# facebookresearch/multimodal

Hardware: NVIDIA H100
Metric: image-text pairs/sec (CLIP ViT-B/16 contrastive pretrain step, bs=512/GPU) (higher is better)
Workload: dtype bf16

## Files before the change

multimodal_b200/csrc/attention.cu:

```cuda
#include "common.cuh"
#include "mmb200_internal.h"
#include <stdlib.h>

namespace mmb {

constexpr int HD = 64;
constexpr int SMAX = 384;

__device__ __forceinline__ uint32_t toff(int r, int c) { return (uint32_t)(r * 128 + ((((c >> 3) ^ (r & 7))) << 4)); }

__device__ __forceinline__ void load_a(uint32_t (&a)[4], uint32_t base, int r0, int c0, int lane) {
  ldsm_x4(a, base + toff(r0 + (lane & 7) + ((lane >> 3) & 1) * 8, c0 + (lane >> 4) * 8));
}
__device__ __forceinline__ void load_b_nk(uint32_t (&b)[4], uint32_t base, int n0, int k0, int lane) {
  ldsm_x4(b, base + toff(n0 + (lane & 7), k0 + (lane >> 3) * 8));
}
__device__ __forceinline__ void load_b_kn(uint32_t (&b)[4], uint32_t base, int k0, int n0, int lane) {
  ldsm_x4_t(b, base + toff(k0 + (lane & 7) + ((lane >> 3) & 1) * 8, n0 + (lane >> 4) * 8));
}

__device__ __forceinline__ void load_tile(uint8_t* dst, const __nv_bfloat16* src, long long ld, int S, int S_pad) {
  for (int i = threadIdx.x; i < S_pad * 8; i += blockDim.x) {
    const int r = i >> 3, ch = i & 7;
    uint4 v = make_uint4(0, 0, 0, 0);
    if (r < S) v = __ldg(reinterpret_cast<const uint4*>(src + (long long)r * ld + ch * 8));
    *reinterpret_cast<uint4*>(dst + toff(r, ch * 8)) = v;
  }
}
__device__ __forceinline__ void load_keymask(uint8_t* dst, const uint8_t* kmask, int S, int S_pad) {
  for (int i = threadIdx.x; i < S_pad; i += blockDim.x) dst[i] = (i < S && (!kmask || kmask[i])) ? 1 : 0;
}

__device__ __forceinline__ float quad_max(float v) {
  v = fmaxf(v, __shfl_xor_sync(0xffffffffu, v, 1));
  return fmaxf(v, __shfl_xor_sync(0xffffffffu, v, 2));
}
__device__ __forceinline__ float quad_sum(float v) {
  v += __shfl_xor_sync(0xffffffffu, v, 1);
  return v + __shfl_xor_sync(0xffffffffu, v, 2);
}

template <bool CAUSAL>
__global__ void __launch_bounds__(256) attn_fwd_kernel(const __nv_bfloat16* __restrict__ qkv,
                                                       __nv_bfloat16* __restrict__ out, float* __restrict__ lse,
                                                       const uint8_t* __restrict__ kmask, int S, int H,
                                                       float scale_log2) {
  extern __shared__ __align__(128) uint8_t asmem[];
  const int S_pad = (S + 15) & ~15;
  const int d = H * HD;
  const long long ld = 3LL * d;
  const int b = blockIdx.x / H, h = blockIdx.x - b * H;
  uint8_t* sQ = asmem;
  uint8_t* sK = sQ + S_pad * 128;
  uint8_t* sV = sK + S_pad * 128;
  uint8_t* sM = sV + S_pad * 128;
  const __nv_bfloat16* base = qkv + (long long)b * S * ld + h * HD;
  load_tile(sQ, base, ld, S, S_pad);
  load_tile(sK, base + d, ld, S, S_pad);
  load_tile(sV, base + 2 * d, ld, S, S_pad);
  load_keymask(sM, kmask ? kmask + (long long)b * S : nullptr, S, S_pad);
  __syncthreads();
  const uint32_t uQ = smem_u32(sQ), uK = smem_u32(sK), uV = smem_u32(sV);
  const int warp = threadIdx.x >> 5, lane = threadIdx.x & 31, nwarps = blockDim.x >> 5;
  const int g = lane >> 2, t = lane & 3;
  const int n_qt = S_pad >> 4;

  for (int qt = warp; qt < n_qt; qt += nwarps) {
    const int q0 = qt * 16;
    uint32_t qa[4][4];
#pragma unroll
    for (int ks = 0; ks < 4; ++ks) load_a(qa[ks], uQ, q0, ks * 16, lane);
    float o[8][4];
#pragma unroll
    for (int i = 0; i < 8; ++i) o[i][0] = o[i][1] = o[i][2] = o[i][3] = 0.f;
    float m0 = -INFINITY, m1 = -INFINITY, l0 = 0.f, l1 = 0.f;
    const int r0 = q0 + g, r1 = r0 + 8;
    const int kv_end = CAUSAL ? min(S, q0 + 16) : S;

    for (int kvb = 0; kvb < kv_end; kvb += 64) {
      const int nt_valid = min(8, (kv_end - kvb + 7) >> 3);
      float s[8][4];
#pragma unroll
      for (int nt = 0; nt < 8; ++nt) {
        s[nt][0] = s[nt][1] = s[nt][2] = s[nt][3] = 0.f;
        if (nt < nt_valid) {
#pragma unroll
          for (int kp = 0; kp < 2; ++kp) {
            uint32_t kb[4];
            load_b_nk(kb, uK, kvb + nt * 8, kp * 32, lane);
            mma16816(s[nt], qa[2 * kp], kb[0], kb[1]);
            mma16816(s[nt], qa[2 * kp + 1], kb[2], kb[3]);
          }
        }
      }
      float mx0 = -INFINITY, mx1 = -INFINITY;
#pragma unroll
      for (int nt = 0; nt < 8; ++nt) {
#pragma unroll
        for (int e = 0; e < 4; ++e) {
          const int col = kvb + nt * 8 + 2 * t + (e & 1);
          const int row = (e < 2) ? r0 : r1;
          float v = s[nt][e] * scale_log2;
          if (col >= kv_end || !sM[col] || (CAUSAL && col > row)) v = -INFINITY;
          s[nt][e] = v;
        }
        mx0 = fmaxf(mx0, fmaxf(s[nt][0], s[nt][1]));
        mx1 = fmaxf(mx1, fmaxf(s[nt][2], s[nt][3]));
      }
      mx0 = quad_max(mx0);
      mx1 = quad_max(mx1);
      const float mn0 = fmaxf(m0, mx0), mn1 = fmaxf(m1, mx1);
      const float b0 = (mn0 == -INFINITY) ? 0.f : mn0, b1 = (mn1 == -INFINITY) ? 0.f : mn1;
      const float c0 = exp2f(m0 - b0), c1 = exp2f(m1 - b1);
      float rs0 = 0.f, rs1 = 0.f;
#pragma unroll
      for (int nt = 0; nt < 8; ++nt) {
        s[nt][0] = exp2f(s[nt][0] - b0);
        s[nt][1] = exp2f(s[nt][1] - b0);
        s[nt][2] = exp2f(s[nt][2] - b1);
        s[nt][3] = exp2f(s[nt][3] - b1);
        rs0 += s[nt][0] + s[nt][1];
        rs1 += s[nt][2] + s[nt][3];
      }
      l0 = l0 * c0 + rs0;
      l1 = l1 * c1 + rs1;
      m0 = mn0;
      m1 = mn1;
#pragma unroll
      for (int i = 0; i < 8; ++i) {
        o[i][0] *= c0; o[i][1] *= c0; o[i][2] *= c1; o[i][3] *= c1;
      }
#pragma unroll
      for (int ks = 0; ks < 4; ++ks) {
        if (2 * ks < nt_valid) {
          uint32_t pa[4];
          pa[0] = pack_bf16x2(s[2 * ks][0], s[2 * ks][1]);
          pa[1] = pack_bf16x2(s[2 * ks][2], s[2 * ks][3]);
          pa[2] = pack_bf16x2(s[2 * ks + 1][0], s[2 * ks + 1][1]);
          pa[3] = pack_bf16x2(s[2 * ks + 1][2], s[2 * ks + 1][3]);
#pragma unroll
          for (int np = 0; np < 4; ++np) {
            uint32_t vb[4];
            load_b_kn(vb, uV, kvb + ks * 16, np * 16, lane);
            mma16816(o[2 * np], pa, vb[0], vb[1]);
            mma16816(o[2 * np + 1], pa, vb[2], vb[3]);
          }
        }
      }
    }
    l0 = quad_sum(l0);
    l1 = quad_sum(l1);
    const float i0 = l0 > 0.f ? 1.f / l0 : 0.f, i1 = l1 > 0.f ? 1.f / l1 : 0.f;
    __nv_bfloat16* orow0 = out + ((long long)b * S + r0) * d + h * HD;
    __nv_bfloat16* orow1 = out + ((long long)b * S + r1) * d + h * HD;
#pragma unroll
    for (int nt = 0; nt < 8; ++nt) {
      if (r0 < S) *reinterpret_cast<uint32_t*>(orow0 + nt * 8 + 2 * t) = pack_bf16x2(o[nt][0] * i0, o[nt][1] * i0);
      if (r1 < S) *reinterpret_cast<uint32_t*>(orow1 + nt * 8 + 2 * t) = pack_bf16x2(o[nt][2] * i1, o[nt][3] * i1);
    }
    if (lse && t == 0) {
      float* lrow = lse + ((long long)b * H + h) * S;
      if (r0 < S) lrow[r0] = (m0 + log2f(l0)) * 0.6931471805599453f;
      if (r1 < S) lrow[r1] = (m1 + log2f(l1)) * 0.6931471805599453f;
    }
  }
}

template <bool CAUSAL>
__global__ void __launch_bounds__(256) attn_bwd_kernel(const __nv_bfloat16* __restrict__ qkv,
                                                       const __nv_bfloat16* __restrict__ out,
                                                       const __nv_bfloat16* __restrict__ dout,
                                                       const float* __restrict__ lse,
                                                       const uint8_t* __restrict__ kmask,
                                                       __nv_bfloat16* __restrict__ dqkv, int S, int H, float scale) {
  extern __shared__ __align__(128) uint8_t asmem[];
  const int S_pad = (S + 15) & ~15;
  const int d = H * HD;
  const long long ld = 3LL * d;
  const int b = blockIdx.x / H, h = blockIdx.x - b * H;
  uint8_t* sQ = asmem;
  uint8_t* sK = sQ + S_pad * 128;
  uint8_t* sV = sK + S_pad * 128;
  uint8_t* sdO = sV + S_pad * 128;
  float* sL = reinterpret_cast<float*>(sdO + S_pad * 128);
  float* sD = sL + S_pad;
  uint8_t* sM = reinterpret_cast<uint8_t*>(sD + S_pad);
  const __nv_bfloat16* base = qkv + (long long)b * S * ld + h * HD;
  const __nv_bfloat16* obase = out + (long long)b * S * d + h * HD;
  const __nv_bfloat16* dobase = dout + (long long)b * S * d + h * HD;
  load_tile(sQ, base, ld, S, S_pad);
  load_tile(sK, base + d, ld, S, S_pad);
  load_tile(sV, base + 2 * d, ld, S, S_pad);
  load_tile(sdO, dobase, d, S, S_pad);
  load_keymask(sM, kmask ? kmask + (long long)b * S : nullptr, S, S_pad);
  const int warp = threadIdx.x >> 5, lane = threadIdx.x & 31, nwarps = blockDim.x >> 5;
  for (int r = warp; r < S_pad; r += nwarps) {
    float acc = 0.f;
    if (r < S) {
      const uint32_t a = *reinterpret_cast<const uint32_t*>(obase + (long long)r * d + lane * 2);
      const uint32_t c = *reinterpret_cast<const uint32_t*>(dobase + (long long)r * d + lane * 2);
      acc = bf16_lo(a) * bf16_lo(c) + bf16_hi(a) * bf16_hi(c);
    }
#pragma unroll
    for (int o = 16; o > 0; o >>= 1) acc += __shfl_xor_sync(0xffffffffu, acc, o);
    if (lane == 0) {
      sD[r] = acc;
      sL[r] = (r < S) ? lse[((long long)b * H + h) * S + r] * 1.4426950408889634f : 0.f;
    }
  }
  __syncthreads();
  const uint32_t uQ = smem_u32(sQ), uK = smem_u32(sK), uV = smem_u32(sV), uO = smem_u32(sdO);
  const int g = lane >> 2, t = lane & 3;
  const int n_t = S_pad >> 4;
  const float scale_log2 = scale * 1.4426950408889634f;
  __nv_bfloat16* dbase = dqkv + (long long)b * S * ld + h * HD;

  for (int j = warp; j < n_t; j += nwarps) {
    const int kv0 = j * 16;
    uint32_t ka[4][4], va[4][4];
#pragma unroll
    for (int ks = 0; ks < 4; ++ks) {
      load_a(ka[ks], uK, kv0, ks * 16, lane);
      load_a(va[ks], uV, kv0, ks * 16, lane);
    }
    float dk[8][4], dv[8][4];
#pragma unroll
    for (int i = 0; i < 8; ++i) {
      dk[i][0] = dk[i][1] = dk[i][2] = dk[i][3] = 0.f;
      dv[i][0] = dv[i][1] = dv[i][2] = dv[i][3] = 0.f;
    }
    const bool kv_ok0 = sM[kv0 + g] != 0, kv_ok1 = sM[kv0 + g + 8] != 0;
    for (int i = CAUSAL ? j : 0; i < n_t; ++i) {
      const int q0 = i * 16;
      float st[2][4], dpt[2][4];
#pragma unroll
      for (int nt = 0; nt < 2; ++nt) {
        st[nt][0] = st[nt][1] = st[nt][2] = st[nt][3] = 0.f;
        dpt[nt][0] = dpt[nt][1] = dpt[nt][2] = dpt[nt][3] = 0.f;
#pragma unroll
        for (int kp = 0; kp < 2; ++kp) {
          uint32_t qb[4], ob[4];
          load_b_nk(qb, uQ, q0 + nt * 8, kp * 32, lane);
          mma16816(st[nt], ka[2 * kp], qb[0], qb[1]);
          mma16816(st[nt], ka[2 * kp + 1], qb[2], qb[3]);
          load_b_nk(ob, uO, q0 + nt * 8, kp * 32, lane);
          mma16816(dpt[nt], va[2 * kp], ob[0], ob[1]);
          mma16816(dpt[nt], va[2 * kp + 1], ob[2], ob[3]);
        }
      }
      float pT[2][4], dsT[2][4];
#pragma unroll
      for (int nt = 0; nt < 2; ++nt)
#pragma unroll
        for (int e = 0; e < 4; ++e) {
          const int kv = kv0 + g + (e >> 1) * 8;
          const int q = q0 + nt * 8 + 2 * t + (e & 1);
          const bool valid = ((e >> 1) ? kv_ok1 : kv_ok0) && (q < S) && (!CAUSAL || kv <= q);
          const float p = valid ? exp2f(st[nt][e] * scale_log2 - sL[q]) : 0.f;
          pT[nt][e] = p;
          dsT[nt][e] = p * (dpt[nt][e] - sD[q]) * scale;
        }
      uint32_t pa[4], dsa[4];
      pa[0] = pack_bf16x2(pT[0][0], pT[0][1]); pa[1] = pack_bf16x2(pT[0][2], pT[0][3]);
      pa[2] = pack_bf16x2(pT[1][0], pT[1][1]); pa[3] = pack_bf16x2(pT[1][2], pT[1][3]);
      dsa[0] = pack_bf16x2(dsT[0][0], dsT[0][1]); dsa[1] = pack_bf16x2(dsT[0][2], dsT[0][3]);
      dsa[2] = pack_bf16x2(dsT[1][0], dsT[1][1]); dsa[3] = pack_bf16x2(dsT[1][2], dsT[1][3]);
#pragma unroll
      for (int np = 0; np < 4; ++np) {
        uint32_t bb[4];
        load_b_kn(bb, uO, q0, np * 16, lane);
        mma16816(dv[2 * np], pa, bb[0], bb[1]);
        mma16816(dv[2 * np + 1], pa, bb[2], bb[3]);
        load_b_kn(bb, uQ, q0, np * 16, lane);
        mma16816(dk[2 * np], dsa, bb[0], bb[1]);
        mma16816(dk[2 * np + 1], dsa, bb[2], bb[3]);
      }
    }
    const int r0 = kv0 + g, r1 = r0 + 8;
#pragma unroll
    for (int nt = 0; nt < 8; ++nt) {
      if (r0 < S) {
        *reinterpret_cast<uint32_t*>(dbase + (long long)r0 * ld + d + nt * 8 + 2 * t) = pack_bf16x2(dk[nt][0], dk[nt][1]);
        *reinterpret_cast<uint32_t*>(dbase + (long long)r0 * ld + 2 * d + nt * 8 + 2 * t) = pack_bf16x2(dv[nt][0], dv[nt][1]);
      }
      if (r1 < S) {
        *reinterpret_cast<uint32_t*>(dbase + (long long)r1 * ld + d + nt * 8 + 2 * t) = pack_bf16x2(dk[nt][2], dk[nt][3]);
        *reinterpret_cast<uint32_t*>(dbase + (long long)r1 * ld + 2 * d + nt * 8 + 2 * t) = pack_bf16x2(dv[nt][2], dv[nt][3]);
      }
    }
  }

  for (int i = warp; i < n_t; i += nwarps) {
    const int q0 = i * 16;
    uint32_t qa[4][4], oa[4][4];
#pragma unroll
    for (int ks = 0; ks < 4; ++ks) {
      load_a(qa[ks], uQ, q0, ks * 16, lane);
      load_a(oa[ks], uO, q0, ks * 16, lane);
    }
    float dq[8][4];
#pragma unroll
    for (int n = 0; n < 8; ++n) dq[n][0] = dq[n][1] = dq[n][2] = dq[n][3] = 0.f;
    const int r0 = q0 + g, r1 = r0 + 8;
    const float L0 = sL[r0], L1 = sL[r1], D0 = sD[r0], D1 = sD[r1];
    const int j_end = CAUSAL ? i + 1 : n_t;
    for (int j = 0; j < j_end; ++j) {
      const int kv0 = j * 16;
      float s[2][4], dp[2][4];
#pragma unroll
      for (int nt = 0; nt < 2; ++nt) {
        s[nt][0] = s[nt][1] = s[nt][2] = s[nt][3] = 0.f;
        dp[nt][0] = dp[nt][1] = dp[nt][2] = dp[nt][3] = 0.f;
#pragma unroll
        for (int kp = 0; kp < 2; ++kp) {
          uint32_t kb[4], vb[4];
          load_b_nk(kb, uK, kv0 + nt * 8, kp * 32, lane);
          mma16816(s[nt], qa[2 * kp], kb[0], kb[1]);
          mma16816(s[nt], qa[2 * kp + 1], kb[2], kb[3]);
          load_b_nk(vb, uV, kv0 + nt * 8, kp * 32, lane);
          mma16816(dp[nt], oa[2 * kp], vb[0], vb[1]);
          mma16816(dp[nt], oa[2 * kp + 1], vb[2], vb[3]);
        }
      }
      float ds[2][4];
#pragma unroll
      for (int nt = 0; nt < 2; ++nt)
#pragma unroll
        for (int e = 0; e < 4; ++e) {
          const int row = (e < 2) ? r0 : r1;
          const int col = kv0 + nt * 8 + 2 * t + (e & 1);
          const bool valid = (row < S) && sM[col] && (!CAUSAL || col <= row);
          const float p = valid ? exp2f(s[nt][e] * scale_log2 - ((e < 2) ? L0 : L1)) : 0.f;
          ds[nt][e] = p * (dp[nt][e] - ((e < 2) ? D0 : D1)) * scale;
        }
      uint32_t dsa[4];
      dsa[0] = pack_bf16x2(ds[0][0], ds[0][1]); dsa[1] = pack_bf16x2(ds[0][2], ds[0][3]);
      dsa[2] = pack_bf16x2(ds[1][0], ds[1][1]); dsa[3] = pack_bf16x2(ds[1][2], ds[1][3]);
#pragma unroll
      for (int np = 0; np < 4; ++np) {
        uint32_t bb[4];
        load_b_kn(bb, uK, kv0, np * 16, lane);
        mma16816(dq[2 * np], dsa, bb[0], bb[1]);
        mma16816(dq[2 * np + 1], dsa, bb[2], bb[3]);
      }
    }
#pragma unroll
    for (int nt = 0; nt < 8; ++nt) {
      if (r0 < S) *reinterpret_cast<uint32_t*>(dbase + (long long)r0 * ld + nt * 8 + 2 * t) = pack_bf16x2(dq[nt][0], dq[nt][1]);
      if (r1 < S) *reinterpret_cast<uint32_t*>(dbase + (long long)r1 * ld + nt * 8 + 2 * t) = pack_bf16x2(dq[nt][2], dq[nt][3]);
    }
  }
}

static int pick_threads(int S) {
  const int n_t = (S + 15) / 16;
  const int per = (n_t + 7) / 8;
  return ((n_t + per - 1) / per) * 32;
}

static int attention_fwd_impl(const void* qkv, void* out, float* lse, const uint8_t* kmask, int B, int S, int H,
                              int causal, float scale, void* stream) {
  if (B <= 0 || S <= 0 || H <= 0 || S > SMAX) return MMB_ERR_UNSUPPORTED;
  const int S_pad = (S + 15) & ~15;
  const int smem = 3 * S_pad * 128 + S_pad;
  const float scale_log2 = scale * 1.4426950408889634f;
  cudaStream_t st = reinterpret_cast<cudaStream_t>(stream);
  auto kfn = causal ? attn_fwd_kernel<true> : attn_fwd_kernel<false>;
  cudaError_t e = cudaFuncSetAttribute(kfn, cudaFuncAttributeMaxDynamicSharedMemorySize, smem);
  if (e != cudaSuccess) return (int)e;
  kfn<<<B * H, pick_threads(S), smem, st>>>((const __nv_bfloat16*)qkv, (__nv_bfloat16*)out, lse, kmask, S, H, scale_log2);
  return (int)cudaGetLastError();
}

static int attention_bwd_impl(const void* qkv, const void* out, const void* dout, const float* lse, void* dqkv,
                              const uint8_t* kmask, int B, int S, int H, int causal, float scale, void* stream) {
  if (B <= 0 || S <= 0 || H <= 0 || S > SMAX) return MMB_ERR_UNSUPPORTED;
  const int S_pad = (S + 15) & ~15;
  const int smem = 4 * S_pad * 128 + 2 * S_pad * 4 + S_pad;
  cudaStream_t st = reinterpret_cast<cudaStream_t>(stream);
  auto kfn = causal ? attn_bwd_kernel<true> : attn_bwd_kernel<false>;
  cudaError_t e = cudaFuncSetAttribute(kfn, cudaFuncAttributeMaxDynamicSharedMemorySize, smem);
  if (e != cudaSuccess) return (int)e;
  kfn<<<B * H, pick_threads(S), smem, st>>>((const __nv_bfloat16*)qkv, (const __nv_bfloat16*)out,
                                            (const __nv_bfloat16*)dout, lse, kmask, (__nv_bfloat16*)dqkv, S, H, scale);
  return (int)cudaGetLastError();
}

}

using namespace mmb;

extern "C" int mmb_attention_bwd_launches(int) { return 1; }

extern "C" int mmb_attention_fwd(const void* qkv, void* out, float* lse, int B, int S, int H, int head_dim, int causal,
                                 float scale, void* stream) {
  if (head_dim != HD) return MMB_ERR_UNSUPPORTED;
  return attention_fwd_impl(qkv, out, lse, nullptr, B, S, H, causal, scale, stream);
}
extern "C" int mmb_attention_fwd_kmask(const void* qkv, void* out, float* lse, const unsigned char* kmask, int B, int S,
// ... 16 lines not shown
```

multimodal_b200/csrc/common.cuh:

```cuda
#pragma once
#include <cuda.h>
#include <cuda_bf16.h>
#include <cuda_runtime.h>
#include <stdint.h>
#include <stdio.h>

namespace mmb {

__device__ __forceinline__ uint32_t smem_u32(const void* p) {
  return static_cast<uint32_t>(__cvta_generic_to_shared(p));
}

__device__ __forceinline__ uint64_t global_timer_ns() {
  uint64_t t;
  asm volatile("mov.u64 %0, %%globaltimer;" : "=l"(t));
  return t;
}

#ifndef MMB_WATCHDOG_NS
#define MMB_WATCHDOG_NS 4000000000ull
#endif

__device__ __forceinline__ void mbar_init(uint64_t* bar, uint32_t count) {
  asm volatile("mbarrier.init.shared::cta.b64 [%0], %1;" ::"r"(smem_u32(bar)), "r"(count) : "memory");
// ... 163 lines not shown
        "+f"(d[32]), "+f"(d[33]), "+f"(d[34]), "+f"(d[35]), "+f"(d[36]), "+f"(d[37]), "+f"(d[38]), "+f"(d[39]),
        "+f"(d[40]), "+f"(d[41]), "+f"(d[42]), "+f"(d[43]), "+f"(d[44]), "+f"(d[45]), "+f"(d[46]), "+f"(d[47]),
        "+f"(d[48]), "+f"(d[49]), "+f"(d[50]), "+f"(d[51]), "+f"(d[52]), "+f"(d[53]), "+f"(d[54]), "+f"(d[55]),
        "+f"(d[56]), "+f"(d[57]), "+f"(d[58]), "+f"(d[59]), "+f"(d[60]), "+f"(d[61]), "+f"(d[62]), "+f"(d[63]),
        "+f"(d[64]), "+f"(d[65]), "+f"(d[66]), "+f"(d[67]), "+f"(d[68]), "+f"(d[69]), "+f"(d[70]), "+f"(d[71]),
        "+f"(d[72]), "+f"(d[73]), "+f"(d[74]), "+f"(d[75]), "+f"(d[76]), "+f"(d[77]), "+f"(d[78]), "+f"(d[79]),
        "+f"(d[80]), "+f"(d[81]), "+f"(d[82]), "+f"(d[83]), "+f"(d[84]), "+f"(d[85]), "+f"(d[86]), "+f"(d[87]),
        "+f"(d[88]), "+f"(d[89]), "+f"(d[90]), "+f"(d[91]), "+f"(d[92]), "+f"(d[93]), "+f"(d[94]), "+f"(d[95]),
        "+f"(d[96]), "+f"(d[97]), "+f"(d[98]), "+f"(d[99]), "+f"(d[100]), "+f"(d[101]), "+f"(d[102]), "+f"(d[103]),
        "+f"(d[104]), "+f"(d[105]), "+f"(d[106]), "+f"(d[107]), "+f"(d[108]), "+f"(d[109]), "+f"(d[110]), "+f"(d[111]),
        "+f"(d[112]), "+f"(d[113]), "+f"(d[114]), "+f"(d[115]), "+f"(d[116]), "+f"(d[117]), "+f"(d[118]), "+f"(d[119]),
        "+f"(d[120]), "+f"(d[121]), "+f"(d[122]), "+f"(d[123]), "+f"(d[124]), "+f"(d[125]), "+f"(d[126]), "+f"(d[127])
      : "l"(adesc), "l"(bdesc), "r"(accumulate), "n"(TA), "n"(TB));
}

template <int N>
__device__ __forceinline__ void setmaxnreg_dec() { asm volatile("setmaxnreg.dec.sync.aligned.u32 %0;" ::"n"(N)); }
template <int N>
__device__ __forceinline__ void setmaxnreg_inc() { asm volatile("setmaxnreg.inc.sync.aligned.u32 %0;" ::"n"(N)); }

__device__ __forceinline__ void ldsm_x4(uint32_t (&r)[4], uint32_t addr) {
  asm volatile("ldmatrix.sync.aligned.m8n8.x4.shared.b16 {%0,%1,%2,%3}, [%4];"
               : "=r"(r[0]), "=r"(r[1]), "=r"(r[2]), "=r"(r[3])
               : "r"(addr));
}
__device__ __forceinline__ void ldsm_x4_t(uint32_t (&r)[4], uint32_t addr) {
  asm volatile("ldmatrix.sync.aligned.m8n8.x4.trans.shared.b16 {%0,%1,%2,%3}, [%4];"
               : "=r"(r[0]), "=r"(r[1]), "=r"(r[2]), "=r"(r[3])
               : "r"(addr));
}
// ... 52 lines not shown
```

Before: 2546.

## Rewrite attention fwd/bwd with TMA loads and wgmma over 64-row query blocks

Replaces the mma.sync/ldmatrix attention kernels with Hopper wgmma (m64n64k16) kernels fed by TMA tile loads into 128B-swizzled shared memory, with per-chunk mbarriers. The grid is split across 64-row query blocks, and in backward across separate key-role and query-role CTAs, instead of one CTA per (batch, head). This gives more parallelism and lets tensor-core work start while later K/V chunks are still arriving. In exchange it adds more redundant K/V loads per CTA, serialised wgmma waits with no overlap between steps, and host-side tensor-map creation on every call.

```diff
diff --git a/multimodal_b200/csrc/attention.cu b/multimodal_b200/csrc/attention.cu
--- a/multimodal_b200/csrc/attention.cu
+++ b/multimodal_b200/csrc/attention.cu
@@ -6,29 +6,18 @@
 
 constexpr int HD = 64;
 constexpr int SMAX = 384;
-
-__device__ __forceinline__ uint32_t toff(int r, int c) { return (uint32_t)(r * 128 + ((((c >> 3) ^ (r & 7))) << 4)); }
-
-__device__ __forceinline__ void load_a(uint32_t (&a)[4], uint32_t base, int r0, int c0, int lane) {
-  ldsm_x4(a, base + toff(r0 + (lane & 7) + ((lane >> 3) & 1) * 8, c0 + (lane >> 4) * 8));
-}
-__device__ __forceinline__ void load_b_nk(uint32_t (&b)[4], uint32_t base, int n0, int k0, int lane) {
-  ldsm_x4(b, base + toff(n0 + (lane & 7), k0 + (lane >> 3) * 8));
-}
-__device__ __forceinline__ void load_b_kn(uint32_t (&b)[4], uint32_t base, int k0, int n0, int lane) {
-  ldsm_x4_t(b, base + toff(k0 + (lane & 7) + ((lane >> 3) & 1) * 8, n0 + (lane >> 4) * 8));
-}
-
-__device__ __forceinline__ void load_tile(uint8_t* dst, const __nv_bfloat16* src, long long ld, int S, int S_pad) {
-  for (int i = threadIdx.x; i < S_pad * 8; i += blockDim.x) {
-    const int r = i >> 3, ch = i & 7;
-    uint4 v = make_uint4(0, 0, 0, 0);
-    if (r < S) v = __ldg(reinterpret_cast<const uint4*>(src + (long long)r * ld + ch * 8));
-    *reinterpret_cast<uint4*>(dst + toff(r, ch * 8)) = v;
-  }
-}
-__device__ __forceinline__ void load_keymask(uint8_t* dst, const uint8_t* kmask, int S, int S_pad) {
-  for (int i = threadIdx.x; i < S_pad; i += blockDim.x) dst[i] = (i < S && (!kmask || kmask[i])) ? 1 : 0;
+constexpr int TROWS = 64;
+constexpr int TILE_BYTES = TROWS * HD * 2;
+constexpr int MAX_CHUNKS = SMAX / TROWS;
+constexpr float LOG2E = 1.4426950408889634f;
+
+__device__ __forceinline__ uint64_t desc_kmajor(const uint8_t* tile) { return make_smem_desc_sw128(smem_u32(tile), 16, 1024); }
+__device__ __forceinline__ uint64_t desc_mnmajor(const uint8_t* tile) { return make_smem_desc_sw128(smem_u32(tile), TILE_BYTES, 1024); }
+constexpr uint64_t KSTEP_K = 32 >> 4;
+constexpr uint64_t KSTEP_MN = 2048 >> 4;
+
+__device__ __forceinline__ uint8_t* align1024(uint8_t* p) {
+  return p + ((1024u - (smem_u32(p) & 1023u)) & 1023u);
 }
 
 __device__ __forceinline__ float quad_max(float v) {
@@ -40,349 +29,342 @@
   return v + __shfl_xor_sync(0xffffffffu, v, 2);
 }
 
+__device__ __forceinline__ void mma_abt(float (&acc)[32], const uint8_t* a, const uint8_t* b) {
+  const uint64_t ad = desc_kmajor(a), bd = desc_kmajor(b);
+#pragma unroll
+  for (int k = 0; k < 4; ++k) wgmma_m64n64k16_ss<0, 0>(acc, ad + k * KSTEP_K, bd + k * KSTEP_K, k > 0 ? 1u : 0u);
+}
+__device__ __forceinline__ void mma_pb(float (&acc)[32], const uint32_t (&p)[4][4], const uint8_t* b) {
+  const uint64_t bd = desc_mnmajor(b);
+#pragma unroll
+  for (int k = 0; k < 4; ++k) wgmma_m64n64k16_rs<1>(acc, p[k], bd + k * KSTEP_MN, 1u);
+}
+__device__ __forceinline__ void pack_a(uint32_t (&p)[4][4], const float (&x)[32]) {
+#pragma unroll
+  for (int k = 0; k < 4; ++k)
+#pragma unroll
+    for (int i = 0; i < 4; ++i) p[k][i] = pack_bf16x2(x[8 * k + 2 * i], x[8 * k + 2 * i + 1]);
+}
+
+__device__ __forceinline__ void load_keymask(uint8_t* dst, const uint8_t* kmask, int S, int n) {
+  for (int i = threadIdx.x; i < n; i += blockDim.x) dst[i] = (i < S && (!kmask || kmask[i])) ? 1 : 0;
+}
+
 template <bool CAUSAL>
-__global__ void __launch_bounds__(256) attn_fwd_kernel(const __nv_bfloat16* __restrict__ qkv,
+__global__ void __launch_bounds__(128) attn_fwd_kernel(const __grid_constant__ CUtensorMap tmQKV,
                                                        __nv_bfloat16* __restrict__ out, float* __restrict__ lse,
                                                        const uint8_t* __restrict__ kmask, int S, int H,
                                                        float scale_log2) {
-  extern __shared__ __align__(128) uint8_t asmem[];
-  const int S_pad = (S + 15) & ~15;
+  extern __shared__ uint8_t smem_raw[];
+  uint8_t* smem = align1024(smem_raw);
+  const int nblk = (S + TROWS - 1) / TROWS;
+  const int bh = blockIdx.x / nblk, qb = blockIdx.x - bh * nblk;
+  const int b = bh / H, h = bh - b * H;
   const int d = H * HD;
-  const long long ld = 3LL * d;
-  const int b = blockIdx.x / H, h = blockIdx.x - b * H;
-  uint8_t* sQ = asmem;
-  uint8_t* sK = sQ + S_pad * 128;
-  uint8_t* sV = sK + S_pad * 128;
-  uint8_t* sM = sV + S_pad * 128;
-  const __nv_bfloat16* base = qkv + (long long)b * S * ld + h * HD;
-  load_tile(sQ, base, ld, S, S_pad);
-  load_tile(sK, base + d, ld, S, S_pad);
-  load_tile(sV, base + 2 * d, ld, S, S_pad);
-  load_keymask(sM, kmask ? kmask + (long long)b * S : nullptr, S, S_pad);
+  const int q0 = qb * TROWS;
+  const int kv_end = CAUSAL ? min(S, q0 + TROWS) : S;
+  const int nkc = (kv_end + TROWS - 1) / TROWS;
+  uint8_t* sQ = smem;
+  uint8_t* sK = sQ + TILE_BYTES;
+  uint8_t* sV = sK + nblk * TILE_BYTES;
+  uint64_t* bar = reinterpret_cast<uint64_t*>(sV + nblk * TILE_BYTES);
+  uint8_t* sM = reinterpret_cast<uint8_t*>(bar + MAX_CHUNKS);
+
+  if (threadIdx.x == 0) {
+    tma_prefetch_desc(&tmQKV);
+    for (int c = 0; c < nkc; ++c) mbar_init(&bar[c], 1);
+    fence_mbar_init();
+    for (int c = 0; c < nkc; ++c) {
+      mbar_arrive_expect_tx(&bar[c], (c == 0 ? 3 : 2) * TILE_BYTES);
+      if (c == 0) tma_load_3d(&tmQKV, &bar[0], sQ, h * HD, q0, b);
+      tma_load_3d(&tmQKV, &bar[c], sK + c * TILE_BYTES, d + h * HD, c * TROWS, b);
+      tma_load_3d(&tmQKV, &bar[c], sV + c * TILE_BYTES, 2 * d + h * HD, c * TROWS, b);
+    }
+  }
+  load_keymask(sM, kmask ? kmask + (long long)b * S : nullptr, S, nkc * TROWS);
   __syncthreads();
-  const uint32_t uQ = smem_u32(sQ), uK = smem_u32(sK), uV = smem_u32(sV);
-  const int warp = threadIdx.x >> 5, lane = threadIdx.x & 31, nwarps = blockDim.x >> 5;
-  const int g = lane >> 2, t = lane & 3;
-  const int n_qt = S_pad >> 4;
-
-  for (int qt = warp; qt < n_qt; qt += nwarps) {
-    const int q0 = qt * 16;
-    uint32_t qa[4][4];
-#pragma unroll
-    for (int ks = 0; ks < 4; ++ks) load_a(qa[ks], uQ, q0, ks * 16, lane);
-    float o[8][4];
-#pragma unroll
-    for (int i = 0; i < 8; ++i) o[i][0] = o[i][1] = o[i][2] = o[i][3] = 0.f;
-    float m0 = -INFINITY, m1 = -INFINITY, l0 = 0.f, l1 = 0.f;
-    const int r0 = q0 + g, r1 = r0 + 8;
-    const int kv_end = CAUSAL ? min(S, q0 + 16) : S;
-
-    for (int kvb = 0; kvb < kv_end; kvb += 64) {
-      const int nt_valid = min(8, (kv_end - kvb + 7) >> 3);
-      float s[8][4];
-#pragma unroll
-      for (int nt = 0; nt < 8; ++nt) {
-        s[nt][0] = s[nt][1] = s[nt][2] = s[nt][3] = 0.f;
-        if (nt < nt_valid) {
-#pragma unroll
-          for (int kp = 0; kp < 2; ++kp) {
-            uint32_t kb[4];
-            load_b_nk(kb, uK, kvb + nt * 8, kp * 32, lane);
-            mma16816(s[nt], qa[2 * kp], kb[0], kb[1]);
-            mma16816(s[nt], qa[2 * kp + 1], kb[2], kb[3]);
-          }
-        }
-      }
-      float mx0 = -INFINITY, mx1 = -INFINITY;
-#pragma unroll
-      for (int nt = 0; nt < 8; ++nt) {
-#pragma unroll
-        for (int e = 0; e < 4; ++e) {
-          const int col = kvb + nt * 8 + 2 * t + (e & 1);
-          const int row = (e < 2) ? r0 : r1;
-          float v = s[nt][e] * scale_log2;
-          if (col >= kv_end || !sM[col] || (CAUSAL && col > row)) v = -INFINITY;
-          s[nt][e] = v;
-        }
-        mx0 = fmaxf(mx0, fmaxf(s[nt][0], s[nt][1]));
-        mx1 = fmaxf(mx1, fmaxf(s[nt][2], s[nt][3]));
-      }
-      mx0 = quad_max(mx0);
-      mx1 = quad_max(mx1);
-      const float mn0 = fmaxf(m0, mx0), mn1 = fmaxf(m1, mx1);
-      const float b0 = (mn0 == -INFINITY) ? 0.f : mn0, b1 = (mn1 == -INFINITY) ? 0.f : mn1;
-      const float c0 = exp2f(m0 - b0), c1 = exp2f(m1 - b1);
-      float rs0 = 0.f, rs1 = 0.f;
-#pragma unroll
-      for (int nt = 0; nt < 8; ++nt) {
-        s[nt][0] = exp2f(s[nt][0] - b0);
-        s[nt][1] = exp2f(s[nt][1] - b0);
-        s[nt][2] = exp2f(s[nt][2] - b1);
-        s[nt][3] = exp2f(s[nt][3] - b1);
-        rs0 += s[nt][0] + s[nt][1];
-        rs1 += s[nt][2] + s[nt][3];
-      }
-      l0 = l0 * c0 + rs0;
-      l1 = l1 * c1 + rs1;
-      m0 = mn0;
-      m1 = mn1;
-#pragma unroll
-      for (int i = 0; i < 8; ++i) {
-        o[i][0] *= c0; o[i][1] *= c0; o[i][2] *= c1; o[i][3] *= c1;
-      }
-#pragma unroll
-      for (int ks = 0; ks < 4; ++ks) {
-        if (2 * ks < nt_valid) {
-          uint32_t pa[4];
-          pa[0] = pack_bf16x2(s[2 * ks][0], s[2 * ks][1]);
-          pa[1] = pack_bf16x2(s[2 * ks][2], s[2 * ks][3]);
-          pa[2] = pack_bf16x2(s[2 * ks + 1][0], s[2 * ks + 1][1]);
-          pa[3] = pack_bf16x2(s[2 * ks + 1][2], s[2 * ks + 1][3]);
-#pragma unroll
-          for (int np = 0; np < 4; ++np) {
-            uint32_t vb[4];
-            load_b_kn(vb, uV, kvb + ks * 16, np * 16, lane);
-            mma16816(o[2 * np], pa, vb[0], vb[1]);
-            mma16816(o[2 * np + 1], pa, vb[2], vb[3]);
-          }
-        }
-      }
-    }
-    l0 = quad_sum(l0);
-    l1 = quad_sum(l1);
-    const float i0 = l0 > 0.f ? 1.f / l0 : 0.f, i1 = l1 > 0.f ? 1.f / l1 : 0.f;
-    __nv_bfloat16* orow0 = out + ((long long)b * S + r0) * d + h * HD;
-    __nv_bfloat16* orow1 = out + ((long long)b * S + r1) * d + h * HD;
-#pragma unroll
-    for (int nt = 0; nt < 8; ++nt) {
-      if (r0 < S) *reinterpret_cast<uint32_t*>(orow0 + nt * 8 + 2 * t) = pack_bf16x2(o[nt][0] * i0, o[nt][1] * i0);
-      if (r1 < S) *reinterpret_cast<uint32_t*>(orow1 + nt * 8 + 2 * t) = pack_bf16x2(o[nt][2] * i1, o[nt][3] * i1);
-    }
-    if (lse && t == 0) {
-      float* lrow = lse + ((long long)b * H + h) * S;
-      if (r0 < S) lrow[r0] = (m0 + log2f(l0)) * 0.6931471805599453f;
-      if (r1 < S) lrow[r1] = (m1 + log2f(l1)) * 0.6931471805599453f;
-    }
+
+  const int warp = threadIdx.x >> 5, lane = threadIdx.x & 31;
+  const int t = lane & 3;
+  const int r0 = q0 + warp * 16 + (lane >> 2), r1 = r0 + 8;
+  float o[32];
+#pragma unroll
+  for (int i = 0; i < 32; ++i) o[i] = 0.f;
+  float m0 = -INFINITY, m1 = -INFINITY, l0 = 0.f, l1 = 0.f;
+
+  for (int c = 0; c < nkc; ++c) {
+    mbar_wait_quiet(&bar[c], 0);
+    float s[32];
+    wgmma_fence();
+    mma_abt(s, sQ, sK + c * TILE_BYTES);
+    wgmma_commit();
+    wgmma_wait<0>();
+    float mx0 = -INFINITY, mx1 = -INFINITY;
+#pragma unroll
+    for (int j = 0; j < 8; ++j) {
+#pragma unroll
+      for (int e = 0; e < 4; ++e) {
+        const int col = c * TROWS + 8 * j + 2 * t + (e & 1);
+        const int row = (e < 2) ? r0 : r1;
+        float v = s[4 * j + e] * scale_log2;
+        if (col >= kv_end || !sM[col] || (CAUSAL && col > row)) v = -INFINITY;
+        s[4 * j + e] = v;
+      }
+      mx0 = fmaxf(mx0, fmaxf(s[4 * j], s[4 * j + 1]));
+      mx1 = fmaxf(mx1, fmaxf(s[4 * j + 2], s[4 * j + 3]));
+    }
+    mx0 = quad_max(mx0);
+    mx1 = quad_max(mx1);
+    const float mn0 = fmaxf(m0, mx0), mn1 = fmaxf(m1, mx1);
+    const float b0 = (mn0 == -INFINITY) ? 0.f : mn0, b1 = (mn1 == -INFINITY) ? 0.f : mn1;
+    const float c0 = exp2f(m0 - b0), c1 = exp2f(m1 - b1);
+    float rs0 = 0.f, rs1 = 0.f;
+#pragma unroll
+    for (int j = 0; j < 8; ++j) {
+      s[4 * j] = exp2f(s[4 * j] - b0);
+      s[4 * j + 1] = exp2f(s[4 * j + 1] - b0);
+      s[4 * j + 2] = exp2f(s[4 * j + 2] - b1);
+      s[4 * j + 3] = exp2f(s[4 * j + 3] - b1);
+      rs0 += s[4 * j] + s[4 * j + 1];
+      rs1 += s[4 * j + 2] + s[4 * j + 3];
+    }
+    l0 = __fadd_rn(__fmul_rn(l0, c0), rs0);
+    l1 = __fadd_rn(__fmul_rn(l1, c1), rs1);
+    m0 = mn0;
+    m1 = mn1;
+#pragma unroll
+    for (int j = 0; j < 8; ++j) {
+      o[4 * j] *= c0; o[4 * j + 1] *= c0; o[4 * j + 2] *= c1; o[4 * j + 3] *= c1;
+    }
+    uint32_t pa[4][4];
+    pack_a(pa, s);
+    wgmma_fence();
+    mma_pb(o, pa, sV + c * TILE_BYTES);
+    wgmma_commit();
+    wgmma_wait<0>();
+  }
+  l0 = quad_sum(l0);
+  l1 = quad_sum(l1);
+  const float i0 = l0 > 0.f ? 1.f / l0 : 0.f, i1 = l1 > 0.f ? 1.f / l1 : 0.f;
+  __nv_bfloat16* orow0 = out + ((long long)b * S + r0) * d + h * HD;
+  __nv_bfloat16* orow1 = out + ((long long)b * S + r1) * d + h * HD;
+#pragma unroll
+  for (int j = 0; j < 8; ++j) {
+    if (r0 < S) *reinterpret_cast<uint32_t*>(orow0 + 8 * j + 2 * t) = pack_bf16x2(o[4 * j] * i0, o[4 * j + 1] * i0);
+    if (r1 < S) *reinterpret_cast<uint32_t*>(orow1 + 8 * j + 2 * t) = pack_bf16x2(o[4 * j + 2] * i1, o[4 * j + 3] * i1);
+  }
+  if (lse && t == 0) {
+    float* lrow = lse + (long long)bh * S;
+    if (r0 < S) lrow[r0] = (m0 + log2f(l0)) * 0.6931471805599453f;
+    if (r1 < S) lrow[r1] = (m1 + log2f(l1)) * 0.6931471805599453f;
   }
 }
 
 template <bool CAUSAL>
-__global__ void __launch_bounds__(256) attn_bwd_kernel(const __nv_bfloat16* __restrict__ qkv,
+__global__ void __launch_bounds__(128) attn_bwd_kernel(const __grid_constant__ CUtensorMap tmQKV,
+                                                       const __grid_constant__ CUtensorMap tmDO,
                                                        const __nv_bfloat16* __restrict__ out,
                                                        const __nv_bfloat16* __restrict__ dout,
                                                        const float* __restrict__ lse,
                                                        const uint8_t* __restrict__ kmask,
                                                        __nv_bfloat16* __restrict__ dqkv, int S, int H, float scale) {
-  extern __shared__ __align__(128) uint8_t asmem[];
-  const int S_pad = (S + 15) & ~15;
+  extern __shared__ uint8_t smem_raw[];
+  uint8_t* smem = align1024(smem_raw);
+  const int nblk = (S + TROWS - 1) / TROWS;
+  const int blk = blockIdx.x % nblk;
+  const bool key_role = ((blockIdx.x / nblk) & 1) == 0;
+  const int bh = blockIdx.x / (2 * nblk);
+  const int b = bh / H, h = bh - b * H;
   const int d = H * HD;
   const long long ld = 3LL * d;
-  const int b = blockIdx.x / H, h = blockIdx.x - b * H;
-  uint8_t* sQ = asmem;
-  uint8_t* sK = sQ + S_pad * 128;
-  uint8_t* sV = sK + S_pad * 128;
-  uint8_t* sdO = sV + S_pad * 128;
-  float* sL = reinterpret_cast<float*>(sdO + S_pad * 128);
-  float* sD = sL + S_pad;
-  uint8_t* sM = reinterpret_cast<uint8_t*>(sD + S_pad);
-  const __nv_bfloat16* base = qkv + (long long)b * S * ld + h * HD;
-  const __nv_bfloat16* obase = out + (long long)b * S * d + h * HD;
-  const __nv_bfloat16* dobase = dout + (long long)b * S * d + h * HD;
-  load_tile(sQ, base, ld, S, S_pad);
-  load_tile(sK, base + d, ld, S, S_pad);
-  load_tile(sV, base + 2 * d, ld, S, S_pad);
-  load_tile(sdO, dobase, d, S, S_pad);
-  load_keymask(sM, kmask ? kmask + (long long)b * S : nullptr, S, S_pad);
-  const int warp = threadIdx.x >> 5, lane = threadIdx.x & 31, nwarps = blockDim.x >> 5;
-  for (int r = warp; r < S_pad; r += nwarps) {
-    float acc = 0.f;
-    if (r < S) {
-      const uint32_t a = *reinterpret_cast<const uint32_t*>(obase + (long long)r * d + lane * 2);
-      const uint32_t c = *reinterpret_cast<const uint32_t*>(dobase + (long long)r * d + lane * 2);
-      acc = bf16_lo(a) * bf16_lo(c) + bf16_hi(a) * bf16_hi(c);
-    }
-#pragma unroll
-    for (int o = 16; o > 0; o >>= 1) acc += __shfl_xor_sync(0xffffffffu, acc, o);
-    if (lane == 0) {
-      sD[r] = acc;
-      sL[r] = (r < S) ? lse[((long long)b * H + h) * S + r] * 1.4426950408889634f : 0.f;
-    }
-  }
+  const int r_own = blk * TROWS;
+  const int c_lo = (CAUSAL && key_role) ? blk : 0;
+  const int c_hi = (CAUSAL && !key_role) ? blk + 1 : nblk;
+  uint8_t* sOwn0 = smem;
+  uint8_t* sOwn1 = sOwn0 + TILE_BYTES;
+  uint8_t* sAll0 = sOwn1 + TILE_BYTES;
+  uint8_t* sAll1 = sAll0 + nblk * TILE_BYTES;
+  uint64_t* bar = reinterpret_cast<uint64_t*>(sAll1 + nblk * TILE_BYTES);
+  float* sL = reinterpret_cast<float*>(bar + MAX_CHUNKS);
+  float* sD = sL + nblk * TROWS;
+  uint8_t* sM = reinterpret_cast<uint8_t*>(sD + nblk * TROWS);
+
+  if (threadIdx.x == 0) {
+    tma_prefetch_desc(&tmQKV);
+    tma_prefetch_desc(&tmDO);
+    for (int c = c_lo; c < c_hi; ++c) mbar_init(&bar[c], 1);
+    fence_mbar_init();
+    const int col_own0 = (key_role ? d : 0) + h * HD;
+    const int col_all0 = (key_role ? 0 : d) + h * HD;
+    for (int c = c_lo; c < c_hi; ++c) {
+      mbar_arrive_expect_tx(&bar[c], (c == c_lo ? 4 : 2) * TILE_BYTES);
+      if (c == c_lo) {
+        tma_load_3d(&tmQKV, &bar[c], sOwn0, col_own0, r_own, b);
+        if (key_role) tma_load_3d(&tmQKV, &bar[c], sOwn1, 2 * d + h * HD, r_own, b);
+        else          tma_load_3d(&tmDO, &bar[c], sOwn1, h * HD, r_own, b);
+      }
+      tma_load_3d(&tmQKV, &bar[c], sAll0 + c * TILE_BYTES, col_all0, c * TROWS, b);
+      if (key_role) tma_load_3d(&tmDO, &bar[c], sAll1 + c * TILE_BYTES, h * HD, c * TROWS, b);
+      else          tma_load_3d(&tmQKV, &bar[c], sAll1 + c * TILE_BYTES, 2 * d + h * HD, c * TROWS, b);
+    }
+  }
+  {
+    const int q_lo = key_role ? c_lo * TROWS : r_own;
+    const int q_hi = key_role ? c_hi * TROWS : r_own + TROWS;
+    const float* lrow = lse + (long long)bh * S;
+    const int t8 = threadIdx.x & 7;
+    for (int r = q_lo + (threadIdx.x >> 3); r < q_hi; r += blockDim.x >> 3) {
+      float acc = 0.f;
+      if (r < S) {
+        const long long off = ((long long)b * S + r) * d + h * HD + 2 * t8;
+        float p[4];
+#pragma unroll
+        for (int k = 0; k < 4; ++k) {
+          const uint32_t a = __ldg(reinterpret_cast<const uint32_t*>(out + off + 16 * k));
+          const uint32_t g = __ldg(reinterpret_cast<const uint32_t*>(dout + off + 16 * k));
+          p[k] = __fmaf_rn(bf16_lo(a), bf16_lo(g), __fmul_rn(bf16_hi(a), bf16_hi(g)));
+        }
+        acc = __fadd_rn(__fadd_rn(p[0], p[2]), __fadd_rn(p[1], p[3]));
+      }
+      acc = __fadd_rn(acc, __shfl_xor_sync(0xffffffffu, acc, 4));
+      acc = __fadd_rn(acc, __shfl_xor_sync(0xffffffffu, acc, 2));
+      acc = __fadd_rn(acc, __shfl_xor_sync(0xffffffffu, acc, 1));
+      if (t8 == 0) {
+        sD[r] = acc;
+        sL[r] = (r < S) ? lrow[r] * LOG2E : 0.f;
+      }
+    }
+  }
+  load_keymask(sM, kmask ? kmask + (long long)b * S : nullptr, S, nblk * TROWS);
   __syncthreads();
-  const uint32_t uQ = smem_u32(sQ), uK = smem_u32(sK), uV = smem_u32(sV), uO = smem_u32(sdO);
-  const int g = lane >> 2, t = lane & 3;
-  const int n_t = S_pad >> 4;
-  const float scale_log2 = scale * 1.4426950408889634f;
+
+  const int warp = threadIdx.x >> 5, lane = threadIdx.x & 31;
+  const int t = lane & 3;
+  const int r0 = r_own + warp * 16 + (lane >> 2), r1 = r0 + 8;
+  const float scale_log2 = scale * LOG2E;
   __nv_bfloat16* dbase = dqkv + (long long)b * S * ld + h * HD;
 
-  for (int j = warp; j < n_t; j += nwarps) {
-    const int kv0 = j * 16;
-    uint32_t ka[4][4], va[4][4];
-#pragma unroll
-    for (int ks = 0; ks < 4; ++ks) {
-      load_a(ka[ks], uK, kv0, ks * 16, lane);
-      load_a(va[ks], uV, kv0, ks * 16, lane);
-    }
-    float dk[8][4], dv[8][4];
-#pragma unroll
-    for (int i = 0; i < 8; ++i) {
-      dk[i][0] = dk[i][1] = dk[i][2] = dk[i][3] = 0.f;
-      dv[i][0] = dv[i][1] = dv[i][2] = dv[i][3] = 0.f;
-    }
-    const bool kv_ok0 = sM[kv0 + g] != 0, kv_ok1 = sM[kv0 + g + 8] != 0;
-    for (int i = CAUSAL ? j : 0; i < n_t; ++i) {
-      const int q0 = i * 16;
-      float st[2][4], dpt[2][4];
-#pragma unroll
-      for (int nt = 0; nt < 2; ++nt) {
-        st[nt][0] = st[nt][1] = st[nt][2] = st[nt][3] = 0.f;
-        dpt[nt][0] = dpt[nt][1] = dpt[nt][2] = dpt[nt][3] = 0.f;
-#pragma unroll
-        for (int kp = 0; kp < 2; ++kp) {
-          uint32_t qb[4], ob[4];
-          load_b_nk(qb, uQ, q0 + nt * 8, kp * 32, lane);
-          mma16816(st[nt], ka[2 * kp], qb[0], qb[1]);
-          mma16816(st[nt], ka[2 * kp + 1], qb[2], qb[3]);
-          load_b_nk(ob, uO, q0 + nt * 8, kp * 32, lane);
-          mma16816(dpt[nt], va[2 * kp], ob[0], ob[1]);
-          mma16816(dpt[nt], va[2 * kp + 1], ob[2], ob[3]);
+  if (key_role) {
+    float dk[32], dv[32];
+#pragma unroll
+    for (int i = 0; i < 32; ++i) dk[i] = dv[i] = 0.f;
+    const bool ok0 = sM[r0] != 0, ok1 = sM[r1] != 0;
+    for (int c = c_lo; c < c_hi; ++c) {
+      mbar_wait_quiet(&bar[c], 0);
+      const uint8_t* tQ = sAll0 + c * TILE_BYTES;
+      const uint8_t* tdO = sAll1 + c * TILE_BYTES;
+      float st[32], dpt[32];
+      wgmma_fence();
+      mma_abt(st, sOwn0, tQ);
+      mma_abt(dpt, sOwn1, tdO);
+      wgmma_commit();
+      wgmma_wait<0>();
+#pragma unroll
+      for (int j = 0; j < 8; ++j)
+#pragma unroll
+        for (int e = 0; e < 4; ++e) {
+          const int kv = (e < 2) ? r0 : r1;
+          const int q = c * TROWS + 8 * j + 2 * t + (e & 1);
+          const bool valid = ((e < 2) ? ok0 : ok1) && (q < S) && (!CAUSAL || kv <= q);
+          const float p = valid ? exp2f(st[4 * j + e] * scale_log2 - sL[q]) : 0.f;
+          st[4 * j + e] = p;
+          dpt[4 * j + e] = p * (dpt[4 * j + e] - sD[q]) * scale;
         }
-      }
-      float pT[2][4], dsT[2][4];
-#pragma unroll
-      for (int nt = 0; nt < 2; ++nt)
-#pragma unroll
-        for (int e = 0; e < 4; ++e) {
-          const int kv = kv0 + g + (e >> 1) * 8;
-          const int q = q0 + nt * 8 + 2 * t + (e & 1);
-          const bool valid = ((e >> 1) ? kv_ok1 : kv_ok0) && (q < S) && (!CAUSAL || kv <= q);
-          const float p = valid ? exp2f(st[nt][e] * scale_log2 - sL[q]) : 0.f;
-          pT[nt][e] = p;
-          dsT[nt][e] = p * (dpt[nt][e] - sD[q]) * scale;
-        }
-      uint32_t pa[4], dsa[4];
-      pa[0] = pack_bf16x2(pT[0][0], pT[0][1]); pa[1] = pack_bf16x2(pT[0][2], pT[0][3]);
-      pa[2] = pack_bf16x2(pT[1][0], pT[1][1]); pa[3] = pack_bf16x2(pT[1][2], pT[1][3]);
-      dsa[0] = pack_bf16x2(dsT[0][0], dsT[0][1]); dsa[1] = pack_bf16x2(dsT[0][2], dsT[0][3]);
-      dsa[2] = pack_bf16x2(dsT[1][0], dsT[1][1]); dsa[3] = pack_bf16x2(dsT[1][2], dsT[1][3]);
-#pragma unroll
-      for (int np = 0; np < 4; ++np) {
-        uint32_t bb[4];
-        load_b_kn(bb, uO, q0, np * 16, lane);
-        mma16816(dv[2 * np], pa, bb[0], bb[1]);
-        mma16816(dv[2 * np + 1], pa, bb[2], bb[3]);
-        load_b_kn(bb, uQ, q0, np * 16, lane);
-        mma16816(dk[2 * np], dsa, bb[0], bb[1]);
-        mma16816(dk[2 * np + 1], dsa, bb[2], bb[3]);
-      }
-    }
-    const int r0 = kv0 + g, r1 = r0 + 8;
-#pragma unroll
-    for (int nt = 0; nt < 8; ++nt) {
+      uint32_t pa[4][4], dsa[4][4];
+      pack_a(pa, st);
+      pack_a(dsa, dpt);
+      wgmma_fence();
+      mma_pb(dv, pa, tdO);
+      mma_pb(dk, dsa, tQ);
+      wgmma_commit();
+      wgmma_wait<0>();
+    }
+#pragma unroll
+    for (int j = 0; j < 8; ++j) {
       if (r0 < S) {
-        *reinterpret_cast<uint32_t*>(dbase + (long long)r0 * ld + d + nt * 8 + 2 * t) = pack_bf16x2(dk[nt][0], dk[nt][1]);
-        *reinterpret_cast<uint32_t*>(dbase + (long long)r0 * ld + 2 * d + nt * 8 + 2 * t) = pack_bf16x2(dv[nt][0], dv[nt][1]);
+        *reinterpret_cast<uint32_t*>(dbase + (long long)r0 * ld + d + 8 * j + 2 * t) = pack_bf16x2(dk[4 * j], dk[4 * j + 1]);
+        *reinterpret_cast<uint32_t*>(dbase + (long long)r0 * ld + 2 * d + 8 * j + 2 * t) = pack_bf16x2(dv[4 * j], dv[4 * j + 1]);
       }
       if (r1 < S) {
-        *reinterpret_cast<uint32_t*>(dbase + (long long)r1 * ld + d + nt * 8 + 2 * t) = pack_bf16x2(dk[nt][2], dk[nt][3]);
-        *reinterpret_cast<uint32_t*>(dbase + (long long)r1 * ld + 2 * d + nt * 8 + 2 * t) = pack_bf16x2(dv[nt][2], dv[nt][3]);
-      }
-    }
-  }
-
-  for (int i = warp; i < n_t; i += nwarps) {
-    const int q0 = i * 16;
-    uint32_t qa[4][4], oa[4][4];
-#pragma unroll
-    for (int ks = 0; ks < 4; ++ks) {
-      load_a(qa[ks], uQ, q0, ks * 16, lane);
-      load_a(oa[ks], uO, q0, ks * 16, lane);
-    }
-    float dq[8][4];
-#pragma unroll
-    for (int n = 0; n < 8; ++n) dq[n][0] = dq[n][1] = dq[n][2] = dq[n][3] = 0.f;
-    const int r0 = q0 + g, r1 = r0 + 8;
+        *reinterpret_cast<uint32_t*>(dbase + (long long)r1 * ld + d + 8 * j + 2 * t) = pack_bf16x2(dk[4 * j + 2], dk[4 * j + 3]);
+        *reinterpret_cast<uint32_t*>(dbase + (long long)r1 * ld + 2 * d + 8 * j + 2 * t) = pack_bf16x2(dv[4 * j + 2], dv[4 * j + 3]);
+      }
+    }
+  } else {
+    float dq[32];
+#pragma unroll
+    for (int i = 0; i < 32; ++i) dq[i] = 0.f;
     const float L0 = sL[r0], L1 = sL[r1], D0 = sD[r0], D1 = sD[r1];
-    const int j_end = CAUSAL ? i + 1 : n_t;
-    for (int j = 0; j < j_end; ++j) {
-      const int kv0 = j * 16;
-      float s[2][4], dp[2][4];
-#pragma unroll
-      for (int nt = 0; nt < 2; ++nt) {
-        s[nt][0] = s[nt][1] = s[nt][2] = s[nt][3] = 0.f;
-        dp[nt][0] = dp[nt][1] = dp[nt][2] = dp[nt][3] = 0.f;
-#pragma unroll
-        for (int kp = 0; kp < 2; ++kp) {
-          uint32_t kb[4], vb[4];
-          load_b_nk(kb, uK, kv0 + nt * 8, kp * 32, lane);
-          mma16816(s[nt], qa[2 * kp], kb[0], kb[1]);
-          mma16816(s[nt], qa[2 * kp + 1], kb[2], kb[3]);
-          load_b_nk(vb, uV, kv0 + nt * 8, kp * 32, lane);
-          mma16816(dp[nt], oa[2 * kp], vb[0], vb[1]);
-          mma16816(dp[nt], oa[2 * kp + 1], vb[2], vb[3]);
-        }
-      }
-      float ds[2][4];
-#pragma unroll
-      for (int nt = 0; nt < 2; ++nt)
+    for (int c = c_lo; c < c_hi; ++c) {
+      mbar_wait_quiet(&bar[c], 0);
+      const uint8_t* tK = sAll0 + c * TILE_BYTES;
+      float s[32], dp[32];
+      wgmma_fence();
+      mma_abt(s, sOwn0, tK);
+      mma_abt(dp, sOwn1, sAll1 + c * TILE_BYTES);
+      wgmma_commit();
+      wgmma_wait<0>();
+#pragma unroll
+      for (int j = 0; j < 8; ++j)
 #pragma unroll
         for (int e = 0; e < 4; ++e) {
           const int row = (e < 2) ? r0 : r1;
-          const int col = kv0 + nt * 8 + 2 * t + (e & 1);
+          const int col = c * TROWS + 8 * j + 2 * t + (e & 1);
           const bool valid = (row < S) && sM[col] && (!CAUSAL || col <= row);
-          const float p = valid ? exp2f(s[nt][e] * scale_log2 - ((e < 2) ? L0 : L1)) : 0.f;
-          ds[nt][e] = p * (dp[nt][e] - ((e < 2) ? D0 : D1)) * scale;
+          const float p = valid ? exp2f(s[4 * j + e] * scale_log2 - ((e < 2) ? L0 : L1)) : 0.f;
+          dp[4 * j + e] = p * (dp[4 * j + e] - ((e < 2) ? D0 : D1)) * scale;
         }
-      uint32_t dsa[4];
-      dsa[0] = pack_bf16x2(ds[0][0], ds[0][1]); dsa[1] = pack_bf16x2(ds[0][2], ds[0][3]);
-      dsa[2] = pack_bf16x2(ds[1][0], ds[1][1]); dsa[3] = pack_bf16x2(ds[1][2], ds[1][3]);
-#pragma unroll
-      for (int np = 0; np < 4; ++np) {
-        uint32_t bb[4];
-        load_b_kn(bb, uK, kv0, np * 16, lane);
-        mma16816(dq[2 * np], dsa, bb[0], bb[1]);
-        mma16816(dq[2 * np + 1], dsa, bb[2], bb[3]);
-      }
-    }
-#pragma unroll
-    for (int nt = 0; nt < 8; ++nt) {
-      if (r0 < S) *reinterpret_cast<uint32_t*>(dbase + (long long)r0 * ld + nt * 8 + 2 * t) = pack_bf16x2(dq[nt][0], dq[nt][1]);
-      if (r1 < S) *reinterpret_cast<uint32_t*>(dbase + (long long)r1 * ld + nt * 8 + 2 * t) = pack_bf16x2(dq[nt][2], dq[nt][3]);
-    }
-  }
-}
-
-static int pick_threads(int S) {
-  const int n_t = (S + 15) / 16;
-  const int per = (n_t + 7) / 8;
-  return ((n_t + per - 1) / per) * 32;
+      uint32_t dsa[4][4];
+      pack_a(dsa, dp);
+      wgmma_fence();
+      mma_pb(dq, dsa, tK);
+      wgmma_commit();
+      wgmma_wait<0>();
+    }
+#pragma unroll
+    for (int j = 0; j < 8; ++j) {
+      if (r0 < S) *reinterpret_cast<uint32_t*>(dbase + (long long)r0 * ld + 8 * j + 2 * t) = pack_bf16x2(dq[4 * j], dq[4 * j + 1]);
+      if (r1 < S) *reinterpret_cast<uint32_t*>(dbase + (long long)r1 * ld + 8 * j + 2 * t) = pack_bf16x2(dq[4 * j + 2], dq[4 * j + 3]);
+    }
+  }
+}
+
+static int qkv_map(CUtensorMap* m, const void* p, int B, int S, int cols) {
+  return make_tmap_3d_bf16(m, p, (uint64_t)cols, (uint64_t)S, (uint64_t)B, (uint64_t)cols * 2,
+                           (uint64_t)S * cols * 2, HD, TROWS);
 }
 
 static int attention_fwd_impl(const void* qkv, void* out, float* lse, const uint8_t* kmask, int B, int S, int H,
                               int causal, float scale, void* stream) {
   if (B <= 0 || S <= 0 || H <= 0 || S > SMAX) return MMB_ERR_UNSUPPORTED;
-  const int S_pad = (S + 15) & ~15;
-  const int smem = 3 * S_pad * 128 + S_pad;
-  const float scale_log2 = scale * 1.4426950408889634f;
+  CUtensorMap tm;
+  int rc = qkv_map(&tm, qkv, B, S, 3 * H * HD);
+  if (rc) return rc;
+  const int nblk = (S + TROWS - 1) / TROWS;
+  const int smem = 1024 + (1 + 2 * nblk) * TILE_BYTES + MAX_CHUNKS * 8 + nblk * TROWS;
   cudaStream_t st = reinterpret_cast<cudaStream_t>(stream);
   auto kfn = causal ? attn_fwd_kernel<true> : attn_fwd_kernel<false>;
   cudaError_t e = cudaFuncSetAttribute(kfn, cudaFuncAttributeMaxDynamicSharedMemorySize, smem);
   if (e != cudaSuccess) return (int)e;
-  kfn<<<B * H, pick_threads(S), smem, st>>>((const __nv_bfloat16*)qkv, (__nv_bfloat16*)out, lse, kmask, S, H, scale_log2);
+  kfn<<<B * H * nblk, 128, smem, st>>>(tm, (__nv_bfloat16*)out, lse, kmask, S, H, scale * LOG2E);
   return (int)cudaGetLastError();
 }
 
 static int attention_bwd_impl(const void* qkv, const void* out, const void* dout, const float* lse, void* dqkv,
                               const uint8_t* kmask, int B, int S, int H, int causal, float scale, void* stream) {
   if (B <= 0 || S <= 0 || H <= 0 || S > SMAX) return MMB_ERR_UNSUPPORTED;
-  const int S_pad = (S + 15) & ~15;
-  const int smem = 4 * S_pad * 128 + 2 * S_pad * 4 + S_pad;
+  CUtensorMap tq, tdo;
+  int rc = qkv_map(&tq, qkv, B, S, 3 * H * HD);
+  if (!rc) rc = qkv_map(&tdo, dout, B, S, H * HD);
+  if (rc) return rc;
+  const int nblk = (S + TROWS - 1) / TROWS;
+  const int smem = 1024 + (2 + 2 * nblk) * TILE_BYTES + MAX_CHUNKS * 8 + nblk * TROWS * (4 + 4 + 1);
   cudaStream_t st = reinterpret_cast<cudaStream_t>(stream);
   auto kfn = causal ? attn_bwd_kernel<true> : attn_bwd_kernel<false>;
   cudaError_t e = cudaFuncSetAttribute(kfn, cudaFuncAttributeMaxDynamicSharedMemorySize, smem);
   if (e != cudaSuccess) return (int)e;
-  kfn<<<B * H, pick_threads(S), smem, st>>>((const __nv_bfloat16*)qkv, (const __nv_bfloat16*)out,
-                                            (const __nv_bfloat16*)dout, lse, kmask, (__nv_bfloat16*)dqkv, S, H, scale);
+  kfn<<<B * H * 2 * nblk, 128, smem, st>>>(tq, tdo, (const __nv_bfloat16*)out, (const __nv_bfloat16*)dout, lse, kmask,
+                                          (__nv_bfloat16*)dqkv, S, H, scale);
   return (int)cudaGetLastError();
 }
 
diff --git a/multimodal_b200/csrc/common.cuh b/multimodal_b200/csrc/common.cuh
--- a/multimodal_b200/csrc/common.cuh
+++ b/multimodal_b200/csrc/common.cuh
@@ -201,6 +201,38 @@
       : "l"(adesc), "l"(bdesc), "r"(accumulate), "n"(TA), "n"(TB));
 }
 
+template <int TA, int TB>
+__device__ __forceinline__ void wgmma_m64n64k16_ss(float (&d)[32], uint64_t adesc, uint64_t bdesc, uint32_t accumulate) {
+  asm volatile(
+      "{\n\t.reg .pred p;\n\t"
+      "setp.ne.b32 p, %34, 0;\n\t"
+      "wgmma.mma_async.sync.aligned.m64n64k16.f32.bf16.bf16 "
+      "{%0, %1, %2, %3, %4, %5, %6, %7, %8, %9, %10, %11, %12, %13, %14, %15, "
+      "%16, %17, %18, %19, %20, %21, %22, %23, %24, %25, %26, %27, %28, %29, %30, %31}, "
+      "%32, %33, p, 1, 1, %35, %36;\n\t}"
+      : "+f"(d[0]), "+f"(d[1]), "+f"(d[2]), "+f"(d[3]), "+f"(d[4]), "+f"(d[5]), "+f"(d[6]), "+f"(d[7]),
+        "+f"(d[8]), "+f"(d[9]), "+f"(d[10]), "+f"(d[11]), "+f"(d[12]), "+f"(d[13]), "+f"(d[14]), "+f"(d[15]),
+        "+f"(d[16]), "+f"(d[17]), "+f"(d[18]), "+f"(d[19]), "+f"(d[20]), "+f"(d[21]), "+f"(d[22]), "+f"(d[23]),
+        "+f"(d[24]), "+f"(d[25]), "+f"(d[26]), "+f"(d[27]), "+f"(d[28]), "+f"(d[29]), "+f"(d[30]), "+f"(d[31])
+      : "l"(adesc), "l"(bdesc), "r"(accumulate), "n"(TA), "n"(TB));
+}
+template <int TB>
+__device__ __forceinline__ void wgmma_m64n64k16_rs(float (&d)[32], const uint32_t (&a)[4], uint64_t bdesc,
+                                                   uint32_t accumulate) {
+  asm volatile(
+      "{\n\t.reg .pred p;\n\t"
+      "setp.ne.b32 p, %37, 0;\n\t"
+      "wgmma.mma_async.sync.aligned.m64n64k16.f32.bf16.bf16 "
+      "{%0, %1, %2, %3, %4, %5, %6, %7, %8, %9, %10, %11, %12, %13, %14, %15, "
+      "%16, %17, %18, %19, %20, %21, %22, %23, %24, %25, %26, %27, %28, %29, %30, %31}, "
+      "{%32, %33, %34, %35}, %36, p, 1, 1, %38;\n\t}"
+      : "+f"(d[0]), "+f"(d[1]), "+f"(d[2]), "+f"(d[3]), "+f"(d[4]), "+f"(d[5]), "+f"(d[6]), "+f"(d[7]),
+        "+f"(d[8]), "+f"(d[9]), "+f"(d[10]), "+f"(d[11]), "+f"(d[12]), "+f"(d[13]), "+f"(d[14]), "+f"(d[15]),
+        "+f"(d[16]), "+f"(d[17]), "+f"(d[18]), "+f"(d[19]), "+f"(d[20]), "+f"(d[21]), "+f"(d[22]), "+f"(d[23]),
+        "+f"(d[24]), "+f"(d[25]), "+f"(d[26]), "+f"(d[27]), "+f"(d[28]), "+f"(d[29]), "+f"(d[30]), "+f"(d[31])
+      : "r"(a[0]), "r"(a[1]), "r"(a[2]), "r"(a[3]), "l"(bdesc), "r"(accumulate), "n"(TB));
+}
+
 template <int N>
 __device__ __forceinline__ void setmaxnreg_dec() { asm volatile("setmaxnreg.dec.sync.aligned.u32 %0;" ::"n"(N)); }
 template <int N>
```

New measurement: 2780 (median of 6 runs). 1.09x the previous value.
